# mbzuai-oryx/Video-LLaVA

Measured on NVIDIA H100. Metric: videos/sec (100-frame CLIP encode + 7B 32-tok decode), higher is better.
Workload: dtype bf16

## Files before the change

video-llava_b200/csrc/attention_tc.cu:

```cuda
#include "common.cuh"
#include "kernels.h"

#include <stdlib.h>

namespace vcl {

namespace {

constexpr int VA_WG = 2;
constexpr int VA_THREADS = VA_WG * 128;
constexpr int VA_TILE = 64 * 128;
constexpr int VA_KEY_TILES = 5;
constexpr int VA_OFF_K = 0;
constexpr int VA_OFF_VT = VA_OFF_K + VA_KEY_TILES * VA_TILE;
constexpr int VA_OFF_Q = VA_OFF_VT + VA_KEY_TILES * VA_TILE;
constexpr int VA_OFF_P = VA_OFF_Q + VA_WG * VA_TILE;
constexpr int VA_OFF_BAR = VA_OFF_P + VA_WG * VA_KEY_TILES * VA_TILE;
constexpr int VA_SMEM = VA_OFF_BAR + 64 + 1024;
static_assert(VA_SMEM <= 227 * 1024, "shared memory");

__device__ __forceinline__ uint32_t va_sw128(int row, int chunk) {
  return (uint32_t)row * 128u + (uint32_t)((chunk ^ (row & 7)) << 4);
}

__device__ __forceinline__ void named_bar_sync_wg(int id) { asm volatile("bar.sync %0, 128;" ::"r"(id) : "memory"); }

__global__ void __launch_bounds__(VA_THREADS, 1)
attn_vit_tc_kernel(const __grid_constant__ CUtensorMap tmap, const bf16* __restrict__ qkv, bf16* __restrict__ out,
                   int S, int H, int C) {
  extern __shared__ uint8_t smem_raw[];
  const uint32_t raw_addr = smem_u32(smem_raw);
  const uint32_t pad = ((raw_addr + 1023u) & ~1023u) - raw_addr;
  uint8_t* smem = smem_raw + pad;
  const uint32_t sbase = raw_addr + pad;
  const uint32_t kbar = sbase + VA_OFF_BAR;
  auto qbar = [&](int w) { return sbase + VA_OFF_BAR + 8u * (1 + w); };

  const int frame = blockIdx.x / H, h = blockIdx.x - frame * H;
  const int row0 = frame * S;
  const int wg = threadIdx.x >> 7, t = threadIdx.x & 127, lane = threadIdx.x & 31, wq = t >> 5;
  const int n_qt = (S + 63) / 64;
  const int n_kt = (S + 63) / 64;

  if (threadIdx.x == 0) {
    tma_prefetch_desc(&tmap);
    mbar_init(kbar, 1);
    for (int w = 0; w < VA_WG; ++w) mbar_init(qbar(w), 1);
    mbar_fence_init();
  }
  __syncthreads();
  if (threadIdx.x == 0) {
    mbar_arrive_expect_tx(kbar, n_kt * VA_TILE);
    for (int i = 0; i < n_kt; ++i) tma_load_2d(sbase + VA_OFF_K + i * VA_TILE, &tmap, kbar, C + h * 64, row0 + 64 * i);
    for (int w = 0; w < VA_WG && w < n_qt; ++w) {
      mbar_arrive_expect_tx(qbar(w), VA_TILE);
      tma_load_2d(sbase + VA_OFF_Q + w * VA_TILE, &tmap, qbar(w), h * 64, row0 + 64 * w);
    }
  }
  const bf16* vg = qkv + (long long)row0 * 3 * C + 2 * C + h * 64;
  for (int idx = threadIdx.x; idx < VA_KEY_TILES * 64 * 8; idx += VA_THREADS) {
    const int key = idx % (VA_KEY_TILES * 64), c = idx / (VA_KEY_TILES * 64);
    uint4 v = make_uint4(0u, 0u, 0u, 0u);
    if (key < S) v = *reinterpret_cast<const uint4*>(vg + (long long)key * 3 * C + c * 8);
    const uint32_t w4[4] = {v.x, v.y, v.z, v.w};
    uint8_t* tile = smem + VA_OFF_VT + (key >> 6) * VA_TILE;
    const int kc = (key & 63) >> 3, ke = key & 7;
#pragma unroll
    for (int e = 0; e < 8; ++e) {
      const uint16_t hv = (uint16_t)(e & 1 ? w4[e >> 1] >> 16 : w4[e >> 1] & 0xffffu);
      *reinterpret_cast<uint16_t*>(tile + va_sw128(c * 8 + e, kc) + ke * 2) = hv;
    }
  }
  asm volatile("fence.proxy.async.shared::cta;" ::: "memory");
  __syncthreads();
  mbar_wait(kbar, 0);

  const int r0 = 16 * wq + (lane >> 2), c2 = 2 * (lane & 3);
  const bool tail = S > 256;
  uint8_t* P = smem + VA_OFF_P + wg * VA_KEY_TILES * VA_TILE;
  const uint32_t p_addr = sbase + VA_OFF_P + wg * VA_KEY_TILES * VA_TILE;
  const uint32_t q_addr = sbase + VA_OFF_Q + wg * VA_TILE;
  uint32_t qphase = 0;
  float s[128], s2[16], o[32];
  for (int qt = wg; qt < n_qt; qt += VA_WG) {
    mbar_wait(qbar(wg), qphase);
    qphase ^= 1u;
#pragma unroll
    for (int i = 0; i < 128; ++i) s[i] = 0.f;
#pragma unroll
    for (int i = 0; i < 16; ++i) s2[i] = 0.f;
    wgmma_fence();
#pragma unroll
    for (int k = 0; k < 4; ++k) {
      const uint64_t ad = wgmma_desc_k_sw128(q_addr) + 2u * k;
      wgmma_bf16<256>(s, ad, wgmma_desc_k_sw128(sbase + VA_OFF_K) + 2u * k, k > 0 ? 1u : 0u);
      if (tail) wgmma_bf16<32>(s2, ad, wgmma_desc_k_sw128(sbase + VA_OFF_K + 256 * 128) + 2u * k, k > 0 ? 1u : 0u);
    }
    wgmma_commit();
    wgmma_wait<0>();
    wgmma_fence_regs(s);
    wgmma_fence_regs(s2);
    named_bar_sync_wg(1 + wg);
    if (t == 0 && qt + VA_WG < n_qt) {
      mbar_arrive_expect_tx(qbar(wg), VA_TILE);
      tma_load_2d(q_addr, &tmap, qbar(wg), h * 64, row0 + 64 * (qt + VA_WG));
    }
    auto sc = [&](float x, int key) { return key < S ? bf16r(bf16r(x) * 0.125f) : -INFINITY; };
    float m[2] = {-INFINITY, -INFINITY};
    uint32_t sp[64], sp2[8];
    auto pack_sc = [&](const float* a, int i, int key0) {
      const int hh = i & 1, col = key0 + 8 * (i >> 1) + c2;
      const float x0 = sc(a[2 * i], col), x1 = sc(a[2 * i + 1], col + 1);
      m[hh] = fmaxf(m[hh], fmaxf(x0, x1));
      return pack_bf16x2(x0, x1);
    };
    if (tail) {
#pragma unroll
      for (int i = 0; i < 8; ++i) sp2[i] = pack_sc(s2, i, 256);
    }
#pragma unroll
    for (int i = 0; i < 64; ++i) sp[i] = pack_sc(s, i, 0);
    float l[2] = {0.f, 0.f};
#pragma unroll
    for (int r = 0; r < 2; ++r) {
      m[r] = fmaxf(m[r], __shfl_xor_sync(0xffffffffu, m[r], 1));
      m[r] = fmaxf(m[r], __shfl_xor_sync(0xffffffffu, m[r], 2));
    }
    auto put_p = [&](uint32_t x2, int i, int key0) {
      const int hh = i & 1, row = r0 + 8 * hh, col = key0 + 8 * (i >> 1) + c2;
      const float p0 = exp2f((bf16lo(x2) - m[hh]) * 1.4426950408889634f);
      const float p1 = exp2f((bf16hi(x2) - m[hh]) * 1.4426950408889634f);
      l[hh] += p0 + p1;
      *reinterpret_cast<uint32_t*>(P + (col >> 6) * VA_TILE + va_sw128(row, (col & 63) >> 3) + (col & 7) * 2) =
          pack_bf16x2(p0, p1);
    };
#pragma unroll
    for (int i = 0; i < 64; ++i) put_p(sp[i], i, 0);
    if (tail) {
#pragma unroll
      for (int i = 0; i < 8; ++i) put_p(sp2[i], i, 256);
    }
    asm volatile("fence.proxy.async.shared::cta;" ::: "memory");
    named_bar_sync_wg(1 + wg);
#pragma unroll
    for (int i = 0; i < 32; ++i) o[i] = 0.f;
    wgmma_fence();
#pragma unroll
    for (int kk = 0; kk < 16; ++kk)
      wgmma_bf16<64>(o, wgmma_desc_k_sw128(p_addr + (kk >> 2) * VA_TILE) + 2u * (kk & 3),
                     wgmma_desc_k_sw128(sbase + VA_OFF_VT + (kk >> 2) * VA_TILE) + 2u * (kk & 3), kk > 0 ? 1u : 0u);
    if (tail)
      wgmma_bf16<64>(o, wgmma_desc_k_sw128(p_addr + 4 * VA_TILE), wgmma_desc_k_sw128(sbase + VA_OFF_VT + 4 * VA_TILE), 1u);
    wgmma_commit();
    wgmma_wait<0>();
    wgmma_fence_regs(o);
#pragma unroll
    for (int r = 0; r < 2; ++r) {
      l[r] += __shfl_xor_sync(0xffffffffu, l[r], 1);
      l[r] += __shfl_xor_sync(0xffffffffu, l[r], 2);
    }
#pragma unroll
    for (int hh = 0; hh < 2; ++hh) {
      const int q = qt * 64 + r0 + 8 * hh;
      if (q < S) {
        const float inv = 1.0f / l[hh];
        bf16* dst = out + (long long)(row0 + q) * C + h * 64 + c2;
#pragma unroll
        for (int j = 0; j < 8; ++j)
          *reinterpret_cast<uint32_t*>(dst + 8 * j) = pack_bf16x2(o[4 * j + 2 * hh] * inv, o[4 * j + 2 * hh + 1] * inv);
      }
    }
  }
}

}

int init_attention_tc_kernels() {
  VCL_CUDA_OK(cudaFuncSetAttribute(attn_vit_tc_kernel, cudaFuncAttributeMaxDynamicSharedMemorySize, VA_SMEM));
  return 0;
}

bool attention_vit_tc_supported(int S) {
  const bool off = getenv("VCL_VIT_ATTN_FLASH") != nullptr;
  return !off && S >= 129 && S <= 257;
}

int launch_attention_vit_tc(const bf16* qkv, bf16* out, int n_frames, int S, int H, int C, cudaStream_t stream) {
  VCL_REQUIRE(C == H * 64, "attention_vit_tc: head_dim must be 64");
  VCL_REQUIRE(S >= 129 && S <= 257, "attention_vit_tc: S=%d outside 129..257", S);
  VCL_REQUIRE(((uintptr_t)qkv % 16) == 0 && ((uintptr_t)out % 16) == 0, "attention_vit_tc: pointers must be 16-byte aligned");
  CUtensorMap tm;
  if (make_tmap_2d(&tm, qkv, (long long)n_frames * S, 3LL * C, 3LL * C, 64) != 0) return -2;
  attn_vit_tc_kernel<<<n_frames * H, VA_THREADS, VA_SMEM, stream>>>(tm, qkv, out, S, H, C);
  VCL_CUDA_OK(cudaGetLastError());
  count_launches(1);
  return 0;
}

}
```

video-llava_b200/csrc/gemm_tc.cu:

```cuda
#include "common.cuh"
#include "kernels.h"

#include <cudaTypedefs.h>

namespace vcl {

template <int BLOCK_N>
struct GemmCfg {
  static constexpr int BLOCK_M = 128;
  static constexpr int BLOCK_K = 64;
  static constexpr int A_BYTES = BLOCK_M * BLOCK_K * 2;
  static constexpr int B_BYTES = BLOCK_N * BLOCK_K * 2;
  static constexpr int STAGE_BYTES = A_BYTES + B_BYTES;
  static constexpr int OUT_PITCH = BLOCK_N * 2 + 16;
  static constexpr int OUT_BYTES = BLOCK_M * OUT_PITCH;
  static constexpr int BAR_BYTES = 256;
  static constexpr int STAGES = (BLOCK_N == 256) ? 3 : (BLOCK_N == 128 ? 5 : 8);
  static constexpr int SMEM_BYTES = STAGES * STAGE_BYTES + BAR_BYTES + OUT_BYTES + 1024;
  static_assert((2 * STAGES + 4) * 8 <= BAR_BYTES, "barrier area");
  static_assert(SMEM_BYTES <= 227 * 1024, "shared memory");
};

__device__ __forceinline__ float act_gelu_erf(float x) {
  x = bf16r(x);
  return 0.5f * x * (1.0f + erff(x * 0.70710678118654752f));
}

template <int BLOCK_N, int ACT>
__device__ __forceinline__ void gemm_epilogue_stage(const float (&acc)[BLOCK_N / 2], uint8_t* stg, int lane, int wq,
                                                    int row_base, int n_blk, const bf16* __restrict__ bias, int M,
                                                    int N, const RopeEpilogue& rp) {
  using Cfg = GemmCfg<BLOCK_N>;
  const int r0 = 16 * wq + (lane >> 2);
  const int c2 = 2 * (lane & 3);
  if constexpr (ACT == ACT_ROPE) {
    static_assert(BLOCK_N % 128 == 0, "one head (128 columns) per tile at least");
#pragma unroll
    for (int hh = 0; hh < BLOCK_N / 128; ++hh) {
      const int gh = n_blk * (BLOCK_N / 128) + hh;
      const int which = gh / rp.H;
#pragma unroll
      for (int h = 0; h < 2; ++h) {
        const int r = r0 + 8 * h;
        const int grow = row_base + r;
        int pos;
        if (rp.pack != nullptr) {
          pos = grow < M ? __ldg(pack_row(rp.pack, grow) + 1) : 0;
        } else {
          pos = rp.start_pos + (grow < M ? grow % rp.S : 0);
          if (rp.n_pad != nullptr && grow < M) pos = max(pos - __ldg(rp.n_pad + grow / rp.S), 0);
// ... 81 lines not shown
      }
    }
#pragma unroll (ACT == ACT_ROPE ? 1 : RES_INFLIGHT)
    for (int u = 0; u < RES_INFLIGHT; ++u) {
      const int r = r0 + u * RSTEP;
      if (r >= rows) break;
      const int grow = row_base + r;
      uint4 val = *reinterpret_cast<const uint4*>(stg + r * Cfg::OUT_PITCH + c * 16);
      bf16* dst = C + (long long)grow * ldc + col;
      if constexpr (ACT == ACT_ROPE) {
        const int gh = col >> 7, d = col & 127;
        const int which = gh / rp.H, head = gh - which * rp.H;
        if (which != 0) {
          int gb, col_c;
          if (rp.pack != nullptr) {
            const int2 sp = __ldg(reinterpret_cast<const int2*>(pack_row(rp.pack, grow)));
            gb = __ldg(pack_slot(rp.pack) + sp.x); col_c = sp.y;
          } else {
            gb = grow / rp.S; col_c = rp.start_pos + grow - gb * rp.S;
          }
          dst = (which == 1 ? rp.kcache : rp.vcache) + d +
                (rp.pages.table != nullptr ? kv_paged_off(rp.pages, gb, head, col_c)
                                           : (((long long)gb * rp.H + head) * rp.s_max + col_c) * 128);
        }
      } else if (RES && residual != nullptr) {
        val.x = bf16x2_add(val.x, rr[u].x); val.y = bf16x2_add(val.y, rr[u].y);
        val.z = bf16x2_add(val.z, rr[u].z); val.w = bf16x2_add(val.w, rr[u].w);
      }
      *reinterpret_cast<uint4*>(dst) = val;
    }
  }
}

template <int BLOCK_N, int ACT, int CL>
__global__ void __launch_bounds__(384, 1)
gemm_bf16_tn_kernel(const __grid_constant__ CUtensorMap tmap_a,
                    const __grid_constant__ CUtensorMap tmap_b, bf16* C, long long ldc,
                    const bf16* __restrict__ bias, const bf16* residual, long long ldr, int M,
                    int N, int K, const RopeEpilogue rope) {
  using Cfg = GemmCfg<BLOCK_N>;
  constexpr int STAGES = Cfg::STAGES;

  extern __shared__ uint8_t smem_raw[];
  const uint32_t raw_addr = smem_u32(smem_raw);
  const uint32_t pad = ((raw_addr + 1023u) & ~1023u) - raw_addr;
  uint8_t* smem = smem_raw + pad;
  const uint32_t smem_base = raw_addr + pad;

  const uint32_t bar_base = smem_base + STAGES * Cfg::STAGE_BYTES;
  auto full_bar = [&](int s) { return bar_base + 8u * s; };
  auto empty_bar = [&](int s) { return bar_base + 8u * (STAGES + s); };
  auto staged_bar = [&](int cw) { return bar_base + 8u * (2 * STAGES + cw); };
  auto drained_bar = [&](int cw) { return bar_base + 8u * (2 * STAGES + 2 + cw); };
  uint8_t* stage_out = smem + STAGES * Cfg::STAGE_BYTES + Cfg::BAR_BYTES;

  const int wg = threadIdx.x >> 7;

  if (threadIdx.x == 0) {
    tma_prefetch_desc(&tmap_a);
    tma_prefetch_desc(&tmap_b);
    for (int s = 0; s < STAGES; ++s) {
      mbar_init(full_bar(s), 1);
      mbar_init(empty_bar(s), 2 * CL);
    }
    for (int cw = 0; cw < 2; ++cw) {
      mbar_init(staged_bar(cw), 128);
      mbar_init(drained_bar(cw), STORE_THREADS);
    }
    mbar_fence_init();
  }
  __syncthreads();
  if (CL > 1) cluster_sync_all();

  const int num_m = (M + Cfg::BLOCK_M - 1) / Cfg::BLOCK_M;
  const int num_n = (N + BLOCK_N - 1) / BLOCK_N;
  const int num_k = (K + Cfg::BLOCK_K - 1) / Cfg::BLOCK_K;
  const int cta_rank = CL > 1 ? (int)cluster_ctarank() : 0;
  const int cluster_id = blockIdx.x / CL, n_clusters = gridDim.x / CL;
  const int num_tiles = ((num_m + CL - 1) / CL) * num_n;
  constexpr uint16_t MC_MASK = (uint16_t)((1u << CL) - 1u);
  constexpr int B_SLICE_ROWS = BLOCK_N / CL;

  if (wg == 0) {
    setmaxnreg_dec<56>();
    if (threadIdx.x == 0) {
      int stage = 0;
      uint32_t phase = 0;
      for (int tile = cluster_id; tile < num_tiles; tile += n_clusters) {
        const int m_blk = (tile / num_n) * CL + cta_rank, n_blk = tile % num_n;
        for (int kb = 0; kb < num_k; ++kb) {
          mbar_wait(empty_bar(stage), phase ^ 1u);
          mbar_arrive_expect_tx(full_bar(stage), Cfg::STAGE_BYTES);
          const uint32_t a_dst = smem_base + stage * Cfg::STAGE_BYTES;
          tma_load_2d(a_dst, &tmap_a, full_bar(stage), kb * Cfg::BLOCK_K, m_blk * Cfg::BLOCK_M);
          if (CL == 1) {
            tma_load_2d(a_dst + Cfg::A_BYTES, &tmap_b, full_bar(stage), kb * Cfg::BLOCK_K, n_blk * BLOCK_N);
          } else {
            tma_load_2d_mc(a_dst + Cfg::A_BYTES + cta_rank * B_SLICE_ROWS * 128, &tmap_b,
                           full_bar(stage), kb * Cfg::BLOCK_K, n_blk * BLOCK_N + cta_rank * B_SLICE_ROWS,
                           MC_MASK);
          }
          if (++stage == STAGES) { stage = 0; phase ^= 1u; }
        }
      }
    } else if (threadIdx.x >= 32) {
      const int t = threadIdx.x - 32;
      uint32_t phase = 0;
      for (int tile = cluster_id; tile < num_tiles; tile += n_clusters) {
        const int m_blk = (tile / num_n) * CL + cta_rank, n_blk = tile % num_n;
#pragma unroll 1
        for (int cw = 0; cw < 2; ++cw) {
          mbar_wait(staged_bar(cw), phase);
          gemm_epilogue_store<BLOCK_N, ACT>(stage_out + cw * 64 * Cfg::OUT_PITCH, t, m_blk * Cfg::BLOCK_M + cw * 64,
                                            n_blk, C, ldc, residual, ldr, M, N, rope);
          mbar_arrive(drained_bar(cw));
        }
        phase ^= 1u;
      }
    }
  } else {
    setmaxnreg_inc<224>();
    const int cw = wg - 1;
    const int t = threadIdx.x & 127, lane = threadIdx.x & 31, wq = t >> 5;
    uint8_t* stg = stage_out + cw * 64 * Cfg::OUT_PITCH;
    auto release = [&](int s) {
      if (t == 0) {
        if (CL == 1) {
          mbar_arrive(empty_bar(s));
        } else {
#pragma unroll
          for (int r = 0; r < CL; ++r) mbar_arrive_cluster(mapa_cluster(empty_bar(s), (uint32_t)r));
        }
      }
    };
    float acc[BLOCK_N / 2];
    int stage = 0;
    uint32_t phase = 0, out_phase = 0;
    for (int tile = cluster_id; tile < num_tiles; tile += n_clusters) {
      const int m_blk = (tile / num_n) * CL + cta_rank, n_blk = tile % num_n;
      int prev = -1;
      for (int kb = 0; kb < num_k; ++kb) {
        mbar_wait(full_bar(stage), phase);
        const uint32_t a_addr = smem_base + stage * Cfg::STAGE_BYTES;
        const uint64_t a_desc = wgmma_desc_k_sw128(a_addr + cw * 64 * 128);
        const uint64_t b_desc = wgmma_desc_k_sw128(a_addr + Cfg::A_BYTES);
        wgmma_fence();
#pragma unroll
        for (int k = 0; k < Cfg::BLOCK_K / 16; ++k) {
          wgmma_bf16<BLOCK_N>(acc, a_desc + 2u * k, b_desc + 2u * k, (kb | k) != 0 ? 1u : 0u);
        }
        wgmma_commit();
        wgmma_wait<1>();
        if (prev >= 0) release(prev);
        prev = stage;
        if (++stage == STAGES) { stage = 0; phase ^= 1u; }
      }
      wgmma_wait<0>();
      release(prev);
      wgmma_fence_regs(acc);
      if (tile != cluster_id) {
        mbar_wait(drained_bar(cw), out_phase);
        out_phase ^= 1u;
      }
      gemm_epilogue_stage<BLOCK_N, ACT>(acc, stg, lane, wq, m_blk * Cfg::BLOCK_M + cw * 64, n_blk, bias, M, N, rope);
      mbar_arrive(staged_bar(cw));
    }
  }

  __syncthreads();
  if (CL > 1) cluster_sync_all();
}

static PFN_cuTensorMapEncodeTiled_v12000 g_encode = nullptr;
static int resolve_encode() {
  if (g_encode) return 0;
  void* fn = nullptr;
  cudaDriverEntryPointQueryResult qres;
  cudaError_t e = cudaGetDriverEntryPoint("cuTensorMapEncodeTiled", &fn, cudaEnableDefault, &qres);
  if (e != cudaSuccess || fn == nullptr || qres != cudaDriverEntryPointSuccess) {
    set_last_error("cuTensorMapEncodeTiled is not available from the driver (%s)",
                   cudaGetErrorString(e));
    return -2;
  }
  g_encode = reinterpret_cast<PFN_cuTensorMapEncodeTiled_v12000>(fn);
  return 0;
}

int make_tmap_2d(CUtensorMap* out, const void* ptr, long long rows, long long cols, long long ld,
                 int box_rows) {
  if (resolve_encode() != 0) return -2;
  cuuint64_t gdim[2] = {(cuuint64_t)cols, (cuuint64_t)rows};
  cuuint64_t gstride[1] = {(cuuint64_t)ld * 2};
  cuuint32_t box[2] = {64u, (cuuint32_t)box_rows};
  cuuint32_t estr[2] = {1u, 1u};
  CUresult r = g_encode(out, CU_TENSOR_MAP_DATA_TYPE_BFLOAT16, 2, const_cast<void*>(ptr), gdim,
                        gstride, box, estr, CU_TENSOR_MAP_INTERLEAVE_NONE,
                        CU_TENSOR_MAP_SWIZZLE_128B, CU_TENSOR_MAP_L2_PROMOTION_L2_256B,
                        CU_TENSOR_MAP_FLOAT_OOB_FILL_NONE);
  if (r != CUDA_SUCCESS) {
    set_last_error("cuTensorMapEncodeTiled failed (%d) ptr=%p rows=%lld cols=%lld ld=%lld box=%d",
                   (int)r, ptr, rows, cols, ld, box_rows);
    return -2;
  }
  return 0;
}

static int g_num_sms = 0;
int device_num_sms() {
  if (g_num_sms == 0) {
    int dev = 0;
    cudaGetDevice(&dev);
    cudaDeviceGetAttribute(&g_num_sms, cudaDevAttrMultiProcessorCount, dev);
    if (g_num_sms <= 0) g_num_sms = 132;
  }
  return g_num_sms;
}

template <int BLOCK_N, int ACT, int CL>
static int launch_one(const GemmArgs& g, cudaStream_t stream) {
  using Cfg = GemmCfg<BLOCK_N>;
  auto kern = gemm_bf16_tn_kernel<BLOCK_N, ACT, CL>;
  CUtensorMap ta, tb;
  if (make_tmap_2d(&ta, g.A, g.M, g.K, g.lda, Cfg::BLOCK_M) != 0) return -2;
  if (make_tmap_2d(&tb, g.W, g.N, g.K, g.ldw, BLOCK_N / CL) != 0) return -2;
  const int num_m = (g.M + 127) / 128;
  const int num_tiles = ((num_m + CL - 1) / CL) * ((g.N + BLOCK_N - 1) / BLOCK_N);
  cudaLaunchConfig_t cfg = {};
  cfg.blockDim = dim3(384);
  cfg.dynamicSmemBytes = Cfg::SMEM_BYTES;
  cfg.stream = stream;
  cudaLaunchAttribute attr[1];
  attr[0].id = cudaLaunchAttributeClusterDimension;
  attr[0].val.clusterDim.x = CL;
  attr[0].val.clusterDim.y = 1;
  attr[0].val.clusterDim.z = 1;
  cfg.attrs = attr;
  cfg.numAttrs = CL > 1 ? 1 : 0;
  static int resident = 0;
  if (resident == 0) {
    if (CL > 1) {
      cfg.gridDim = dim3(CL);
      VCL_CUDA_OK(cudaOccupancyMaxActiveClusters(&resident, kern, &cfg));
    }
    if (resident <= 0) resident = device_num_sms() / CL;
  }
  int clusters = resident;
  if (clusters > num_tiles) clusters = num_tiles;
  if (g.max_ctas > 0 && clusters * CL > g.max_ctas) clusters = g.max_ctas / CL > 0 ? g.max_ctas / CL : 1;
  cfg.gridDim = dim3(clusters * CL);
  VCL_CUDA_OK(cudaLaunchKernelEx(&cfg, kern, ta, tb, g.C, (long long)g.ldc, g.bias, g.residual,
                                 (long long)g.ldr, g.M, g.N, g.K, g.rope));
  count_launches(1);
  return 0;
}

template <int BLOCK_N, int ACT>
static int launch_cl(const GemmArgs& g, int cl, cudaStream_t stream) {
  if (BLOCK_N >= 128) {
    if (cl == 4) return launch_one<BLOCK_N, ACT, (BLOCK_N >= 128 ? 4 : 1)>(g, stream);
    if (cl == 2) return launch_one<BLOCK_N, ACT, (BLOCK_N >= 128 ? 2 : 1)>(g, stream);
  }
  return launch_one<BLOCK_N, ACT, 1>(g, stream);
}

template <int BLOCK_N>
static int launch_act(const GemmArgs& g, int cl, cudaStream_t stream) {
  switch (g.act) {
    case ACT_NONE: return launch_cl<BLOCK_N, ACT_NONE>(g, cl, stream);
    case ACT_QGELU: return launch_cl<BLOCK_N, ACT_QGELU>(g, cl, stream);
    case ACT_GELU: return launch_cl<BLOCK_N, ACT_GELU>(g, cl, stream);
    case ACT_SWIGLU: return launch_cl<BLOCK_N, ACT_SWIGLU>(g, cl, stream);
    case ACT_ROPE:
      if constexpr (BLOCK_N >= 128) return launch_cl<BLOCK_N, ACT_ROPE>(g, cl, stream);
      break;
  }
  set_last_error("gemm: unknown activation %d", g.act);
  return -1;
}

template <int BLOCK_N, int ACT>
static int init_one() {
  VCL_CUDA_OK(cudaFuncSetAttribute(gemm_bf16_tn_kernel<BLOCK_N, ACT, 1>,
                                   cudaFuncAttributeMaxDynamicSharedMemorySize,
                                   GemmCfg<BLOCK_N>::SMEM_BYTES));
  if (BLOCK_N >= 128) {
    VCL_CUDA_OK(cudaFuncSetAttribute(gemm_bf16_tn_kernel<BLOCK_N, ACT, (BLOCK_N >= 128 ? 2 : 1)>,
                                     cudaFuncAttributeMaxDynamicSharedMemorySize,
                                     GemmCfg<BLOCK_N>::SMEM_BYTES));
    VCL_CUDA_OK(cudaFuncSetAttribute(gemm_bf16_tn_kernel<BLOCK_N, ACT, (BLOCK_N >= 128 ? 4 : 1)>,
                                     cudaFuncAttributeMaxDynamicSharedMemorySize,
                                     GemmCfg<BLOCK_N>::SMEM_BYTES));
  }
  return 0;
}
template <int BLOCK_N>
static int init_bn() {
  if (init_one<BLOCK_N, ACT_NONE>() || init_one<BLOCK_N, ACT_QGELU>() ||
      init_one<BLOCK_N, ACT_GELU>() || init_one<BLOCK_N, ACT_SWIGLU>()) return -2;
  if constexpr (BLOCK_N >= 128) {
    if (init_one<BLOCK_N, ACT_ROPE>()) return -2;
  }
  return 0;
}
int init_gemm_kernels() {
  if (resolve_encode() != 0) return -2;
  if (init_bn<256>() || init_bn<128>() || init_bn<64>() || init_bn<32>()) return -2;
  return 0;
}

int launch_gemm_bf16_tn(const GemmArgs& g, cudaStream_t stream) {
  VCL_REQUIRE(g.M > 0 && g.N > 0 && g.K > 0, "gemm: empty problem M=%d N=%d K=%d", g.M, g.N, g.K);
  VCL_REQUIRE(g.K % 64 == 0, "gemm: K=%d must be a multiple of 64", g.K);
  VCL_REQUIRE(g.N % 32 == 0, "gemm: N=%d must be a multiple of 32", g.N);
  VCL_REQUIRE(g.lda % 8 == 0 && g.ldw % 8 == 0 && g.ldc % 8 == 0, "gemm: pitches must be x8");
  VCL_REQUIRE(((uintptr_t)g.A % 16) == 0 && ((uintptr_t)g.W % 16) == 0 &&
                  ((uintptr_t)g.C % 16) == 0, "gemm: pointers must be 16-byte aligned");
  VCL_REQUIRE(g.residual == nullptr || (g.ldr % 8 == 0 && ((uintptr_t)g.residual % 16) == 0),
              "gemm: residual must be 16-byte aligned with pitch x8");
  VCL_REQUIRE(g.bias == nullptr || ((uintptr_t)g.bias % 16) == 0, "gemm: bias alignment");
  VCL_REQUIRE(!(g.act == ACT_SWIGLU && g.residual != nullptr), "gemm: swiglu takes no residual");
  if (g.act == ACT_ROPE) {
    const RopeEpilogue& r = g.rope;
    VCL_REQUIRE(r.cos_t && r.sin_t && r.kcache && r.vcache && r.S > 0 && r.H > 0, "gemm: ACT_ROPE needs the RoPE tables and the cache");
    VCL_REQUIRE(g.N == 3 * r.H * 128 && (r.pack != nullptr || g.M % r.S == 0) && r.start_pos + r.S <= r.s_max &&
                    g.bias == nullptr && g.residual == nullptr,
                "gemm: ACT_ROPE shape (N=%d, H=%d, M=%d, S=%d, start %d, cache %d)", g.N, r.H, g.M, r.S, r.start_pos, r.s_max);
    VCL_REQUIRE(((uintptr_t)r.kcache % 16) == 0 && ((uintptr_t)r.vcache % 16) == 0 && ((uintptr_t)r.cos_t % 16) == 0 &&
                    ((uintptr_t)r.sin_t % 16) == 0, "gemm: ACT_ROPE pointers must be 16-byte aligned");
  }
  int bn = g.block_n;
  int cl = g.cluster;
  if (bn == 0) {
    const int sms = device_num_sms();
    const long long mt = (g.M + 127) / 128;
    if (mt == 1) {
      bn = 256;
      while (bn > 32 && (g.N % bn != 0 || g.N / bn < sms)) bn >>= 1;
      if (g.N % bn != 0) bn = 32;
    } else if (g.N % 256 == 0 && mt * (g.N / 256) >= sms && !(g.N <= 1024 && g.K <= 1024)) {
      bn = 256;
    } else {
      bn = (g.N % 128 == 0) ? 128 : (g.N % 64 == 0) ? 64 : 32;
    }
  }
  if (cl == 0) cl = 1;
  if (cl == -2) cl = (bn == 256 || bn == 128) && g.N % bn == 0 ? 2 : 1;
  if (g.act == ACT_ROPE && g.block_n == 0 && bn < 128) bn = 128;
  VCL_REQUIRE(g.act != ACT_ROPE || bn == 128 || bn == 256, "gemm: ACT_ROPE needs 128- or 256-wide tiles (one head = 128 columns), got %d", bn);
  VCL_REQUIRE(cl == 1 || cl == 2 || cl == 4, "gemm: cluster must be 1, 2 or 4 (got %d)", cl);
  switch (bn) {
    case 256: return launch_act<256>(g, cl, stream);
    case 128: return launch_act<128>(g, cl, stream);
    case 64: return launch_act<64>(g, 1, stream);
    case 32: return launch_act<32>(g, 1, stream);
  }
  set_last_error("gemm: unsupported block_n %d", bn);
  return -1;
}

}
```

Baseline: 5.045.

## Make ViT attention persistent and warp-specialized with TMA K/V pipeline and register P

The ViT attention kernel becomes persistent, with the grid capped at the SM count. A dedicated producer warpgroup streams K, V and Q tiles through double-buffered stages and mbarriers, so loads overlap compute across (frame, head) items. V is now loaded by TMA instead of being transposed manually, and the softmax P stays in registers as the wgmma A operand instead of going through shared memory. It also adds a TAIL template, bf16x2 max/scale, and a fast ex2.approx path when the value range allows it, in exchange for more complex synchronisation and slight numeric differences.

```diff
diff --git a/video-llava_b200/csrc/attention_tc.cu b/video-llava_b200/csrc/attention_tc.cu
--- a/video-llava_b200/csrc/attention_tc.cu
+++ b/video-llava_b200/csrc/attention_tc.cu
@@ -3,157 +3,202 @@
 
 #include <stdlib.h>
 
+#include <type_traits>
+
 namespace vcl {
 
 namespace {
 
 constexpr int VA_WG = 2;
-constexpr int VA_THREADS = VA_WG * 128;
+constexpr int VA_THREADS = (VA_WG + 1) * 128;
 constexpr int VA_TILE = 64 * 128;
 constexpr int VA_KEY_TILES = 5;
-constexpr int VA_OFF_K = 0;
-constexpr int VA_OFF_VT = VA_OFF_K + VA_KEY_TILES * VA_TILE;
-constexpr int VA_OFF_Q = VA_OFF_VT + VA_KEY_TILES * VA_TILE;
-constexpr int VA_OFF_P = VA_OFF_Q + VA_WG * VA_TILE;
-constexpr int VA_OFF_BAR = VA_OFF_P + VA_WG * VA_KEY_TILES * VA_TILE;
-constexpr int VA_SMEM = VA_OFF_BAR + 64 + 1024;
+constexpr int VA_STAGES = 2;
+constexpr int VA_Q_SLOTS = 4;
+constexpr int VA_STAGE = 2 * VA_KEY_TILES * VA_TILE;
+constexpr int VA_OFF_Q = VA_STAGES * VA_STAGE;
+constexpr int VA_OFF_BAR = VA_OFF_Q + VA_Q_SLOTS * VA_TILE;
+constexpr int VA_SMEM = VA_OFF_BAR + 128 + 1024;
 static_assert(VA_SMEM <= 227 * 1024, "shared memory");
 
-__device__ __forceinline__ uint32_t va_sw128(int row, int chunk) {
-  return (uint32_t)row * 128u + (uint32_t)((chunk ^ (row & 7)) << 4);
-}
-
-__device__ __forceinline__ void named_bar_sync_wg(int id) { asm volatile("bar.sync %0, 128;" ::"r"(id) : "memory"); }
-
+__device__ __forceinline__ void wgmma_pv(float (&d)[32], uint32_t a0, uint32_t a1, uint32_t a2, uint32_t a3,
+                                         uint64_t bdesc, uint32_t accumulate) {
+  asm volatile(
+      "{\n\t.reg .pred p;\n\tsetp.ne.b32 p, %37, 0;\n\t"
+      "wgmma.mma_async.sync.aligned.m64n64k16.f32.bf16.bf16 {%0, %1, %2, %3, %4, %5, %6, %7, %8, %9, %10, %11, %12, %13, %14, %15, %16, %17, %18, %19, %20, %21, %22, %23, %24, %25, %26, %27, %28, %29, %30, %31}, {%32, %33, %34, %35}, %36, p, 1, 1, 1;\n\t}"
+      : "+f"(d[0]), "+f"(d[1]), "+f"(d[2]), "+f"(d[3]), "+f"(d[4]), "+f"(d[5]), "+f"(d[6]), "+f"(d[7]), "+f"(d[8]), "+f"(d[9]), "+f"(d[10]), "+f"(d[11]), "+f"(d[12]), "+f"(d[13]), "+f"(d[14]), "+f"(d[15]), "+f"(d[16]), "+f"(d[17]), "+f"(d[18]), "+f"(d[19]), "+f"(d[20]), "+f"(d[21]), "+f"(d[22]), "+f"(d[23]), "+f"(d[24]), "+f"(d[25]), "+f"(d[26]), "+f"(d[27]), "+f"(d[28]), "+f"(d[29]), "+f"(d[30]), "+f"(d[31])
+      : "r"(a0), "r"(a1), "r"(a2), "r"(a3), "l"(bdesc), "r"(accumulate));
+}
+
+__device__ __forceinline__ uint32_t bf16x2_max(uint32_t a, uint32_t b) {
+  __nv_bfloat162 r = __hmax2(*reinterpret_cast<__nv_bfloat162*>(&a), *reinterpret_cast<__nv_bfloat162*>(&b));
+  return *reinterpret_cast<uint32_t*>(&r);
+}
+
+__device__ __forceinline__ uint32_t bf16x2_min(uint32_t a, uint32_t b) {
+  __nv_bfloat162 r = __hmin2(*reinterpret_cast<__nv_bfloat162*>(&a), *reinterpret_cast<__nv_bfloat162*>(&b));
+  return *reinterpret_cast<uint32_t*>(&r);
+}
+__device__ __forceinline__ float ex2_approx(float x) {
+  float y;
+  asm("ex2.approx.ftz.f32 %0, %1;" : "=f"(y) : "f"(x));
+  return y;
+}
+
+template <bool TAIL>
 __global__ void __launch_bounds__(VA_THREADS, 1)
-attn_vit_tc_kernel(const __grid_constant__ CUtensorMap tmap, const bf16* __restrict__ qkv, bf16* __restrict__ out,
-                   int S, int H, int C) {
+attn_vit_tc_kernel(const __grid_constant__ CUtensorMap tmap, bf16* __restrict__ out, int S, int H, int C,
+                   int n_items) {
   extern __shared__ uint8_t smem_raw[];
   const uint32_t raw_addr = smem_u32(smem_raw);
   const uint32_t pad = ((raw_addr + 1023u) & ~1023u) - raw_addr;
-  uint8_t* smem = smem_raw + pad;
   const uint32_t sbase = raw_addr + pad;
-  const uint32_t kbar = sbase + VA_OFF_BAR;
-  auto qbar = [&](int w) { return sbase + VA_OFF_BAR + 8u * (1 + w); };
-
-  const int frame = blockIdx.x / H, h = blockIdx.x - frame * H;
-  const int row0 = frame * S;
-  const int wg = threadIdx.x >> 7, t = threadIdx.x & 127, lane = threadIdx.x & 31, wq = t >> 5;
+  auto kv_full = [&](int st) { return sbase + VA_OFF_BAR + 8u * st; };
+  auto kv_empty = [&](int st) { return sbase + VA_OFF_BAR + 8u * (VA_STAGES + st); };
+  auto q_full = [&](int sl) { return sbase + VA_OFF_BAR + 8u * (2 * VA_STAGES + sl); };
+  auto q_empty = [&](int sl) { return sbase + VA_OFF_BAR + 8u * (2 * VA_STAGES + VA_Q_SLOTS + sl); };
+
+  constexpr int n_kv = TAIL ? 5 : 4;
   const int n_qt = (S + 63) / 64;
-  const int n_kt = (S + 63) / 64;
+  const int lane = threadIdx.x & 31;
 
   if (threadIdx.x == 0) {
-    tma_prefetch_desc(&tmap);
-    mbar_init(kbar, 1);
-    for (int w = 0; w < VA_WG; ++w) mbar_init(qbar(w), 1);
+    for (int i = 0; i < VA_STAGES; ++i) {
+      mbar_init(kv_full(i), 1);
+      mbar_init(kv_empty(i), 2 * 4);
+    }
+    for (int i = 0; i < VA_Q_SLOTS; ++i) {
+      mbar_init(q_full(i), 1);
+      mbar_init(q_empty(i), 4);
+    }
     mbar_fence_init();
   }
   __syncthreads();
-  if (threadIdx.x == 0) {
-    mbar_arrive_expect_tx(kbar, n_kt * VA_TILE);
-    for (int i = 0; i < n_kt; ++i) tma_load_2d(sbase + VA_OFF_K + i * VA_TILE, &tmap, kbar, C + h * 64, row0 + 64 * i);
-    for (int w = 0; w < VA_WG && w < n_qt; ++w) {
-      mbar_arrive_expect_tx(qbar(w), VA_TILE);
-      tma_load_2d(sbase + VA_OFF_Q + w * VA_TILE, &tmap, qbar(w), h * 64, row0 + 64 * w);
-    }
+
+  if (threadIdx.x >= VA_WG * 128) {
+    setmaxnreg_dec<40>();
+    if (threadIdx.x == VA_WG * 128) {
+      const int n_mine = (n_items - (int)blockIdx.x + (int)gridDim.x - 1) / (int)gridDim.x;
+      tma_prefetch_desc(&tmap);
+      for (int j = 0, g = 0; j < n_mine; ++j) {
+        const int item = blockIdx.x + j * gridDim.x, frame = item / H, h = item - frame * H, row0 = frame * S;
+        const int st = j & 1;
+        if (j >= VA_STAGES) mbar_wait(kv_empty(st), ((j >> 1) - 1) & 1);
+        const uint32_t k_addr = sbase + st * VA_STAGE, v_addr = k_addr + VA_KEY_TILES * VA_TILE;
+        mbar_arrive_expect_tx(kv_full(st), 2 * n_kv * VA_TILE);
+        for (int i = 0; i < n_kv; ++i) {
+          tma_load_2d(k_addr + i * VA_TILE, &tmap, kv_full(st), C + h * 64, row0 + 64 * i);
+          tma_load_2d(v_addr + i * VA_TILE, &tmap, kv_full(st), 2 * C + h * 64, row0 + 64 * i);
+        }
+        for (int qt = 0; qt < n_qt; ++qt, ++g) {
+          const int sl = g & (VA_Q_SLOTS - 1);
+          if (g >= VA_Q_SLOTS) mbar_wait(q_empty(sl), ((g >> 2) - 1) & 1);
+          mbar_arrive_expect_tx(q_full(sl), VA_TILE);
+          tma_load_2d(sbase + VA_OFF_Q + sl * VA_TILE, &tmap, q_full(sl), h * 64, row0 + 64 * qt);
+        }
+      }
+    }
+    return;
   }
-  const bf16* vg = qkv + (long long)row0 * 3 * C + 2 * C + h * 64;
-  for (int idx = threadIdx.x; idx < VA_KEY_TILES * 64 * 8; idx += VA_THREADS) {
-    const int key = idx % (VA_KEY_TILES * 64), c = idx / (VA_KEY_TILES * 64);
-    uint4 v = make_uint4(0u, 0u, 0u, 0u);
-    if (key < S) v = *reinterpret_cast<const uint4*>(vg + (long long)key * 3 * C + c * 8);
-    const uint32_t w4[4] = {v.x, v.y, v.z, v.w};
-    uint8_t* tile = smem + VA_OFF_VT + (key >> 6) * VA_TILE;
-    const int kc = (key & 63) >> 3, ke = key & 7;
-#pragma unroll
-    for (int e = 0; e < 8; ++e) {
-      const uint16_t hv = (uint16_t)(e & 1 ? w4[e >> 1] >> 16 : w4[e >> 1] & 0xffffu);
-      *reinterpret_cast<uint16_t*>(tile + va_sw128(c * 8 + e, kc) + ke * 2) = hv;
-    }
-  }
-  asm volatile("fence.proxy.async.shared::cta;" ::: "memory");
-  __syncthreads();
-  mbar_wait(kbar, 0);
-
+
+  setmaxnreg_inc<232>();
+  const int n_tiles = (n_items - (int)blockIdx.x + (int)gridDim.x - 1) / (int)gridDim.x * n_qt;
+  const int wg = threadIdx.x >> 7, t = threadIdx.x & 127, wq = t >> 5;
   const int r0 = 16 * wq + (lane >> 2), c2 = 2 * (lane & 3);
-  const bool tail = S > 256;
-  uint8_t* P = smem + VA_OFF_P + wg * VA_KEY_TILES * VA_TILE;
-  const uint32_t p_addr = sbase + VA_OFF_P + wg * VA_KEY_TILES * VA_TILE;
-  const uint32_t q_addr = sbase + VA_OFF_Q + wg * VA_TILE;
-  uint32_t qphase = 0;
-  float s[128], s2[16], o[32];
-  for (int qt = wg; qt < n_qt; qt += VA_WG) {
-    mbar_wait(qbar(wg), qphase);
-    qphase ^= 1u;
-#pragma unroll
-    for (int i = 0; i < 128; ++i) s[i] = 0.f;
-#pragma unroll
-    for (int i = 0; i < 16; ++i) s2[i] = 0.f;
+  for (int g = wg; g < n_tiles; g += VA_WG) {
+    const int j = g / n_qt, qt = g - j * n_qt;
+    const int item = blockIdx.x + j * gridDim.x, frame = item / H, h = item - frame * H, row0 = frame * S;
+    const int st = j & 1, sl = g & (VA_Q_SLOTS - 1);
+    const uint32_t k_addr = sbase + st * VA_STAGE, v_addr = k_addr + VA_KEY_TILES * VA_TILE;
+    const uint32_t q_addr = sbase + VA_OFF_Q + sl * VA_TILE;
+    mbar_wait(kv_full(st), (j >> 1) & 1);
+    mbar_wait(q_full(sl), (g >> 2) & 1);
+    float s[128], s2[TAIL ? 16 : 1];
     wgmma_fence();
 #pragma unroll
     for (int k = 0; k < 4; ++k) {
       const uint64_t ad = wgmma_desc_k_sw128(q_addr) + 2u * k;
-      wgmma_bf16<256>(s, ad, wgmma_desc_k_sw128(sbase + VA_OFF_K) + 2u * k, k > 0 ? 1u : 0u);
-      if (tail) wgmma_bf16<32>(s2, ad, wgmma_desc_k_sw128(sbase + VA_OFF_K + 256 * 128) + 2u * k, k > 0 ? 1u : 0u);
+      wgmma_bf16<256>(s, ad, wgmma_desc_k_sw128(k_addr) + 2u * k, k > 0 ? 1u : 0u);
+      if constexpr (TAIL) wgmma_bf16<32>(s2, ad, wgmma_desc_k_sw128(k_addr + 256 * 128) + 2u * k, k > 0 ? 1u : 0u);
     }
     wgmma_commit();
     wgmma_wait<0>();
     wgmma_fence_regs(s);
-    wgmma_fence_regs(s2);
-    named_bar_sync_wg(1 + wg);
-    if (t == 0 && qt + VA_WG < n_qt) {
-      mbar_arrive_expect_tx(qbar(wg), VA_TILE);
-      tma_load_2d(q_addr, &tmap, qbar(wg), h * 64, row0 + 64 * (qt + VA_WG));
-    }
-    auto sc = [&](float x, int key) { return key < S ? bf16r(bf16r(x) * 0.125f) : -INFINITY; };
-    float m[2] = {-INFINITY, -INFINITY};
+    if constexpr (TAIL) wgmma_fence_regs(s2);
+    __syncwarp();
+    if (lane == 0) mbar_arrive(q_empty(sl));
+
+    constexpr int S_MIN = TAIL ? 257 : 129;
     uint32_t sp[64], sp2[8];
+    uint32_t mx[2] = {0xff80ff80u, 0xff80ff80u};
+    uint32_t mn[2] = {0x7f807f80u, 0x7f807f80u};
     auto pack_sc = [&](const float* a, int i, int key0) {
       const int hh = i & 1, col = key0 + 8 * (i >> 1) + c2;
-      const float x0 = sc(a[2 * i], col), x1 = sc(a[2 * i + 1], col + 1);
-      m[hh] = fmaxf(m[hh], fmaxf(x0, x1));
-      return pack_bf16x2(x0, x1);
+      uint32_t x2 = bf16x2_mul(pack_bf16x2(a[2 * i], a[2 * i + 1]), 0x3e003e00u);
+      mn[hh] = bf16x2_min(mn[hh], x2);
+      if (key0 + 8 * (i >> 1) + 7 >= S_MIN) {
+        if (col >= S) x2 = (x2 & 0xffff0000u) | 0xff80u;
+        if (col + 1 >= S) x2 = (x2 & 0xffffu) | 0xff800000u;
+      }
+      mx[hh] = bf16x2_max(mx[hh], x2);
+      return x2;
     };
-    if (tail) {
+    if constexpr (TAIL) {
 #pragma unroll
       for (int i = 0; i < 8; ++i) sp2[i] = pack_sc(s2, i, 256);
     }
 #pragma unroll
     for (int i = 0; i < 64; ++i) sp[i] = pack_sc(s, i, 0);
-    float l[2] = {0.f, 0.f};
+    float m[2], l[2] = {0.f, 0.f};
+    bool near = true;
 #pragma unroll
     for (int r = 0; r < 2; ++r) {
+      m[r] = fmaxf(bf16lo(mx[r]), bf16hi(mx[r]));
       m[r] = fmaxf(m[r], __shfl_xor_sync(0xffffffffu, m[r], 1));
       m[r] = fmaxf(m[r], __shfl_xor_sync(0xffffffffu, m[r], 2));
-    }
-    auto put_p = [&](uint32_t x2, int i, int key0) {
-      const int hh = i & 1, row = r0 + 8 * hh, col = key0 + 8 * (i >> 1) + c2;
-      const float p0 = exp2f((bf16lo(x2) - m[hh]) * 1.4426950408889634f);
-      const float p1 = exp2f((bf16hi(x2) - m[hh]) * 1.4426950408889634f);
+      near = near && (fminf(bf16lo(mn[r]), bf16hi(mn[r])) - m[r]) * 1.4426950408889634f >= -126.f;
+    }
+    auto p_of = [&](uint32_t x2, int i, auto bare) {
+      const int hh = i & 1;
+      const float x0 = (bf16lo(x2) - m[hh]) * 1.4426950408889634f;
+      const float x1 = (bf16hi(x2) - m[hh]) * 1.4426950408889634f;
+      const float p0 = bare ? ex2_approx(x0) : exp2f(x0), p1 = bare ? ex2_approx(x1) : exp2f(x1);
       l[hh] += p0 + p1;
-      *reinterpret_cast<uint32_t*>(P + (col >> 6) * VA_TILE + va_sw128(row, (col & 63) >> 3) + (col & 7) * 2) =
-          pack_bf16x2(p0, p1);
+      return pack_bf16x2(p0, p1);
     };
-#pragma unroll
-    for (int i = 0; i < 64; ++i) put_p(sp[i], i, 0);
-    if (tail) {
-#pragma unroll
-      for (int i = 0; i < 8; ++i) put_p(sp2[i], i, 256);
-    }
-    asm volatile("fence.proxy.async.shared::cta;" ::: "memory");
-    named_bar_sync_wg(1 + wg);
-#pragma unroll
-    for (int i = 0; i < 32; ++i) o[i] = 0.f;
+    if (qt * 64 + 16 * wq < S) {
+      if (__all_sync(0xffffffffu, near)) {
+#pragma unroll
+        for (int i = 0; i < 64; ++i) sp[i] = p_of(sp[i], i, std::true_type{});
+        if constexpr (TAIL) {
+#pragma unroll
+          for (int i = 0; i < 8; ++i) sp2[i] = p_of(sp2[i], i, std::true_type{});
+        }
+      } else {
+#pragma unroll
+        for (int i = 0; i < 64; ++i) sp[i] = p_of(sp[i], i, std::false_type{});
+        if constexpr (TAIL) {
+#pragma unroll
+          for (int i = 0; i < 8; ++i) sp2[i] = p_of(sp2[i], i, std::false_type{});
+        }
+      }
+    }
+
+    float o[32];
     wgmma_fence();
 #pragma unroll
     for (int kk = 0; kk < 16; ++kk)
-      wgmma_bf16<64>(o, wgmma_desc_k_sw128(p_addr + (kk >> 2) * VA_TILE) + 2u * (kk & 3),
-                     wgmma_desc_k_sw128(sbase + VA_OFF_VT + (kk >> 2) * VA_TILE) + 2u * (kk & 3), kk > 0 ? 1u : 0u);
-    if (tail)
-      wgmma_bf16<64>(o, wgmma_desc_k_sw128(p_addr + 4 * VA_TILE), wgmma_desc_k_sw128(sbase + VA_OFF_VT + 4 * VA_TILE), 1u);
+      wgmma_pv(o, sp[4 * kk], sp[4 * kk + 1], sp[4 * kk + 2], sp[4 * kk + 3],
+               wgmma_desc_k_sw128(v_addr + (kk >> 2) * VA_TILE + (kk & 3) * 16 * 128), kk > 0 ? 1u : 0u);
+    if constexpr (TAIL) wgmma_pv(o, sp2[0], sp2[1], sp2[2], sp2[3], wgmma_desc_k_sw128(v_addr + 4 * VA_TILE), 1u);
     wgmma_commit();
     wgmma_wait<0>();
     wgmma_fence_regs(o);
+    if (g + VA_WG >= n_tiles || (g + VA_WG) / n_qt != j) {
+      __syncwarp();
+      if (lane == 0) mbar_arrive(kv_empty(st));
+    }
+
 #pragma unroll
     for (int r = 0; r < 2; ++r) {
       l[r] += __shfl_xor_sync(0xffffffffu, l[r], 1);
@@ -166,8 +211,9 @@
         const float inv = 1.0f / l[hh];
         bf16* dst = out + (long long)(row0 + q) * C + h * 64 + c2;
 #pragma unroll
-        for (int j = 0; j < 8; ++j)
-          *reinterpret_cast<uint32_t*>(dst + 8 * j) = pack_bf16x2(o[4 * j + 2 * hh] * inv, o[4 * j + 2 * hh + 1] * inv);
+        for (int j8 = 0; j8 < 8; ++j8)
+          *reinterpret_cast<uint32_t*>(dst + 8 * j8) =
+              pack_bf16x2(o[4 * j8 + 2 * hh] * inv, o[4 * j8 + 2 * hh + 1] * inv);
       }
     }
   }
@@ -176,7 +222,8 @@
 }
 
 int init_attention_tc_kernels() {
-  VCL_CUDA_OK(cudaFuncSetAttribute(attn_vit_tc_kernel, cudaFuncAttributeMaxDynamicSharedMemorySize, VA_SMEM));
+  VCL_CUDA_OK(cudaFuncSetAttribute(attn_vit_tc_kernel<false>, cudaFuncAttributeMaxDynamicSharedMemorySize, VA_SMEM));
+  VCL_CUDA_OK(cudaFuncSetAttribute(attn_vit_tc_kernel<true>, cudaFuncAttributeMaxDynamicSharedMemorySize, VA_SMEM));
   return 0;
 }
 
@@ -191,7 +238,15 @@
   VCL_REQUIRE(((uintptr_t)qkv % 16) == 0 && ((uintptr_t)out % 16) == 0, "attention_vit_tc: pointers must be 16-byte aligned");
   CUtensorMap tm;
   if (make_tmap_2d(&tm, qkv, (long long)n_frames * S, 3LL * C, 3LL * C, 64) != 0) return -2;
-  attn_vit_tc_kernel<<<n_frames * H, VA_THREADS, VA_SMEM, stream>>>(tm, qkv, out, S, H, C);
+  int dev = 0, sms = 0;
+  VCL_CUDA_OK(cudaGetDevice(&dev));
+  VCL_CUDA_OK(cudaDeviceGetAttribute(&sms, cudaDevAttrMultiProcessorCount, dev));
+  const int items = n_frames * H;
+  const int grid = items < sms ? items : sms;
+  if (S > 256)
+    attn_vit_tc_kernel<true><<<grid, VA_THREADS, VA_SMEM, stream>>>(tm, out, S, H, C, items);
+  else
+    attn_vit_tc_kernel<false><<<grid, VA_THREADS, VA_SMEM, stream>>>(tm, out, S, H, C, items);
   VCL_CUDA_OK(cudaGetLastError());
   count_launches(1);
   return 0;
```

New measurement: 5.142 (median of 6 runs). 1.9% higher.

## Add 64-row unit schedule for GEMM and M-fast tile order for small M

Applied to the files above, without the earlier changes.

Adds an opt-in GEMM schedule (cluster=-1) that splits work into 64-row by BLOCK_N units, divides them evenly across CTAs and pairs consecutive units per pass, loading a second B strip when the pair crosses strips. For small M (num_m<=4) the default path now walks tiles M-fastest so that CTAs sharing a weight strip run together, and the 256-wide tile choice drops its K condition. An environment override for tile and cluster is also added. The unit path is meant to reduce wave-quantization tail imbalance, at the cost of more complex barrier bookkeeping and extra B traffic.

```diff
diff --git a/video-llava_b200/csrc/gemm_tc.cu b/video-llava_b200/csrc/gemm_tc.cu
--- a/video-llava_b200/csrc/gemm_tc.cu
+++ b/video-llava_b200/csrc/gemm_tc.cu
@@ -2,20 +2,23 @@
 #include "kernels.h"
 
 #include <cudaTypedefs.h>
+#include <cstdio>
+#include <cstdlib>
 
 namespace vcl {
 
-template <int BLOCK_N>
+template <int BLOCK_N, bool UNITS = false>
 struct GemmCfg {
   static constexpr int BLOCK_M = 128;
   static constexpr int BLOCK_K = 64;
   static constexpr int A_BYTES = BLOCK_M * BLOCK_K * 2;
   static constexpr int B_BYTES = BLOCK_N * BLOCK_K * 2;
-  static constexpr int STAGE_BYTES = A_BYTES + B_BYTES;
+  static constexpr int STAGE_BYTES = A_BYTES + (UNITS ? 2 : 1) * B_BYTES;
   static constexpr int OUT_PITCH = BLOCK_N * 2 + 16;
   static constexpr int OUT_BYTES = BLOCK_M * OUT_PITCH;
   static constexpr int BAR_BYTES = 256;
-  static constexpr int STAGES = (BLOCK_N == 256) ? 3 : (BLOCK_N == 128 ? 5 : 8);
+  static constexpr int STAGES = UNITS ? (227 * 1024 - BAR_BYTES - OUT_BYTES - 1024) / STAGE_BYTES
+                                      : (BLOCK_N == 256) ? 3 : (BLOCK_N == 128 ? 5 : 8);
   static constexpr int SMEM_BYTES = STAGES * STAGE_BYTES + BAR_BYTES + OUT_BYTES + 1024;
   static_assert((2 * STAGES + 4) * 8 <= BAR_BYTES, "barrier area");
   static_assert(SMEM_BYTES <= 227 * 1024, "shared memory");
@@ -163,13 +166,14 @@
   }
 }
 
-template <int BLOCK_N, int ACT, int CL>
+template <int BLOCK_N, int ACT, int CL, bool UNITS = false>
 __global__ void __launch_bounds__(384, 1)
 gemm_bf16_tn_kernel(const __grid_constant__ CUtensorMap tmap_a,
                     const __grid_constant__ CUtensorMap tmap_b, bf16* C, long long ldc,
                     const bf16* __restrict__ bias, const bf16* residual, long long ldr, int M,
                     int N, int K, const RopeEpilogue rope) {
-  using Cfg = GemmCfg<BLOCK_N>;
+  static_assert(!UNITS || CL == 1, "the unit schedule runs without a cluster");
+  using Cfg = GemmCfg<BLOCK_N, UNITS>;
   constexpr int STAGES = Cfg::STAGES;
 
   extern __shared__ uint8_t smem_raw[];
@@ -211,21 +215,62 @@
   const int num_tiles = ((num_m + CL - 1) / CL) * num_n;
   constexpr uint16_t MC_MASK = (uint16_t)((1u << CL) - 1u);
   constexpr int B_SLICE_ROWS = BLOCK_N / CL;
+  const int num_rb = (M + 63) / 64;
+  const long long num_units = (long long)num_rb * num_n;
+  const int it_begin = UNITS ? (int)(blockIdx.x * num_units / gridDim.x) : cluster_id;
+  const int it_end = UNITS ? (int)((blockIdx.x + 1) * num_units / gridDim.x) : num_tiles;
+  const int it_step = UNITS ? 2 : n_clusters;
+  const bool m_fast = CL == 1 && num_m <= 4;
+  struct Pass {
+    int row0, row1, strip0, strip1;
+    bool has1, two_b;
+    __device__ int row(int cw) const { return cw ? row1 : row0; }
+    __device__ int strip(int cw) const { return cw ? strip1 : strip0; }
+  };
+  auto pass_of = [&](int it) {
+    Pass p;
+    if constexpr (UNITS) {
+      p.has1 = it + 1 < it_end;
+      p.strip0 = it / num_rb;
+      p.row0 = (it - p.strip0 * num_rb) * 64;
+      p.strip1 = (it + 1) / num_rb;
+      p.row1 = (it + 1 - p.strip1 * num_rb) * 64;
+      p.two_b = p.has1 && p.strip1 != p.strip0;
+    } else if (m_fast) {
+      p.row0 = (it % num_m) * Cfg::BLOCK_M; p.row1 = p.row0 + 64;
+      p.strip0 = p.strip1 = it / num_m;
+      p.has1 = true; p.two_b = false;
+    } else {
+      const int m_blk = (it / num_n) * CL + cta_rank;
+      p.row0 = m_blk * Cfg::BLOCK_M; p.row1 = p.row0 + 64;
+      p.strip0 = p.strip1 = it % num_n;
+      p.has1 = true; p.two_b = false;
+    }
+    return p;
+  };
 
   if (wg == 0) {
     setmaxnreg_dec<56>();
     if (threadIdx.x == 0) {
       int stage = 0;
       uint32_t phase = 0;
-      for (int tile = cluster_id; tile < num_tiles; tile += n_clusters) {
-        const int m_blk = (tile / num_n) * CL + cta_rank, n_blk = tile % num_n;
+      for (int it = it_begin; it < it_end; it += it_step) {
+        const Pass p = pass_of(it);
+        const int n_blk = p.strip0;
+        const uint32_t bytes = UNITS ? (p.has1 ? 2 : 1) * (Cfg::A_BYTES / 2) + (p.two_b ? 2 : 1) * Cfg::B_BYTES
+                                     : Cfg::STAGE_BYTES;
         for (int kb = 0; kb < num_k; ++kb) {
           mbar_wait(empty_bar(stage), phase ^ 1u);
-          mbar_arrive_expect_tx(full_bar(stage), Cfg::STAGE_BYTES);
+          mbar_arrive_expect_tx(full_bar(stage), bytes);
           const uint32_t a_dst = smem_base + stage * Cfg::STAGE_BYTES;
-          tma_load_2d(a_dst, &tmap_a, full_bar(stage), kb * Cfg::BLOCK_K, m_blk * Cfg::BLOCK_M);
+          tma_load_2d(a_dst, &tmap_a, full_bar(stage), kb * Cfg::BLOCK_K, p.row0);
+          if (UNITS && p.has1)
+            tma_load_2d(a_dst + Cfg::A_BYTES / 2, &tmap_a, full_bar(stage), kb * Cfg::BLOCK_K, p.row1);
           if (CL == 1) {
             tma_load_2d(a_dst + Cfg::A_BYTES, &tmap_b, full_bar(stage), kb * Cfg::BLOCK_K, n_blk * BLOCK_N);
+            if (p.two_b)
+              tma_load_2d(a_dst + Cfg::A_BYTES + Cfg::B_BYTES, &tmap_b, full_bar(stage), kb * Cfg::BLOCK_K,
+                          p.strip1 * BLOCK_N);
           } else {
             tma_load_2d_mc(a_dst + Cfg::A_BYTES + cta_rank * B_SLICE_ROWS * 128, &tmap_b,
                            full_bar(stage), kb * Cfg::BLOCK_K, n_blk * BLOCK_N + cta_rank * B_SLICE_ROWS,
@@ -237,13 +282,13 @@
     } else if (threadIdx.x >= 32) {
       const int t = threadIdx.x - 32;
       uint32_t phase = 0;
-      for (int tile = cluster_id; tile < num_tiles; tile += n_clusters) {
-        const int m_blk = (tile / num_n) * CL + cta_rank, n_blk = tile % num_n;
+      for (int it = it_begin; it < it_end; it += it_step) {
+        const Pass p = pass_of(it);
 #pragma unroll 1
-        for (int cw = 0; cw < 2; ++cw) {
+        for (int cw = 0; cw < (p.has1 ? 2 : 1); ++cw) {
           mbar_wait(staged_bar(cw), phase);
-          gemm_epilogue_store<BLOCK_N, ACT>(stage_out + cw * 64 * Cfg::OUT_PITCH, t, m_blk * Cfg::BLOCK_M + cw * 64,
-                                            n_blk, C, ldc, residual, ldr, M, N, rope);
+          gemm_epilogue_store<BLOCK_N, ACT>(stage_out + cw * 64 * Cfg::OUT_PITCH, t, p.row(cw), p.strip(cw), C, ldc,
+                                            residual, ldr, M, N, rope);
           mbar_arrive(drained_bar(cw));
         }
         phase ^= 1u;
@@ -267,14 +312,23 @@
     float acc[BLOCK_N / 2];
     int stage = 0;
     uint32_t phase = 0, out_phase = 0;
-    for (int tile = cluster_id; tile < num_tiles; tile += n_clusters) {
-      const int m_blk = (tile / num_n) * CL + cta_rank, n_blk = tile % num_n;
+    for (int it = it_begin; it < it_end; it += it_step) {
+      const Pass p = pass_of(it);
+      if (cw == 1 && !p.has1) {
+        for (int kb = 0; kb < num_k; ++kb) {
+          mbar_wait(full_bar(stage), phase);
+          release(stage);
+          if (++stage == STAGES) { stage = 0; phase ^= 1u; }
+        }
+        continue;
+      }
+      const uint32_t b_off = Cfg::A_BYTES + (p.two_b && cw == 1 ? Cfg::B_BYTES : 0);
       int prev = -1;
       for (int kb = 0; kb < num_k; ++kb) {
         mbar_wait(full_bar(stage), phase);
         const uint32_t a_addr = smem_base + stage * Cfg::STAGE_BYTES;
         const uint64_t a_desc = wgmma_desc_k_sw128(a_addr + cw * 64 * 128);
-        const uint64_t b_desc = wgmma_desc_k_sw128(a_addr + Cfg::A_BYTES);
+        const uint64_t b_desc = wgmma_desc_k_sw128(a_addr + b_off);
         wgmma_fence();
 #pragma unroll
         for (int k = 0; k < Cfg::BLOCK_K / 16; ++k) {
@@ -289,11 +343,11 @@
       wgmma_wait<0>();
       release(prev);
       wgmma_fence_regs(acc);
-      if (tile != cluster_id) {
+      if (it != it_begin) {
         mbar_wait(drained_bar(cw), out_phase);
         out_phase ^= 1u;
       }
-      gemm_epilogue_stage<BLOCK_N, ACT>(acc, stg, lane, wq, m_blk * Cfg::BLOCK_M + cw * 64, n_blk, bias, M, N, rope);
+      gemm_epilogue_stage<BLOCK_N, ACT>(acc, stg, lane, wq, p.row(cw), p.strip(cw), bias, M, N, rope);
       mbar_arrive(staged_bar(cw));
     }
   }
@@ -347,15 +401,16 @@
   return g_num_sms;
 }
 
-template <int BLOCK_N, int ACT, int CL>
+template <int BLOCK_N, int ACT, int CL, bool UNITS = false>
 static int launch_one(const GemmArgs& g, cudaStream_t stream) {
-  using Cfg = GemmCfg<BLOCK_N>;
-  auto kern = gemm_bf16_tn_kernel<BLOCK_N, ACT, CL>;
+  using Cfg = GemmCfg<BLOCK_N, UNITS>;
+  auto kern = gemm_bf16_tn_kernel<BLOCK_N, ACT, CL, UNITS>;
   CUtensorMap ta, tb;
-  if (make_tmap_2d(&ta, g.A, g.M, g.K, g.lda, Cfg::BLOCK_M) != 0) return -2;
+  if (make_tmap_2d(&ta, g.A, g.M, g.K, g.lda, UNITS ? 64 : Cfg::BLOCK_M) != 0) return -2;
   if (make_tmap_2d(&tb, g.W, g.N, g.K, g.ldw, BLOCK_N / CL) != 0) return -2;
   const int num_m = (g.M + 127) / 128;
-  const int num_tiles = ((num_m + CL - 1) / CL) * ((g.N + BLOCK_N - 1) / BLOCK_N);
+  const int num_n = (g.N + BLOCK_N - 1) / BLOCK_N;
+  const int num_tiles = UNITS ? (int)(((long long)(g.M + 63) / 64 * num_n + 1) / 2) : ((num_m + CL - 1) / CL) * num_n;
   cudaLaunchConfig_t cfg = {};
   cfg.blockDim = dim3(384);
   cfg.dynamicSmemBytes = Cfg::SMEM_BYTES;
@@ -387,6 +442,9 @@
 
 template <int BLOCK_N, int ACT>
 static int launch_cl(const GemmArgs& g, int cl, cudaStream_t stream) {
+  if constexpr (BLOCK_N == 128 || BLOCK_N == 64) {
+    if (cl == -1) return launch_one<BLOCK_N, ACT, 1, true>(g, stream);
+  }
   if (BLOCK_N >= 128) {
     if (cl == 4) return launch_one<BLOCK_N, ACT, (BLOCK_N >= 128 ? 4 : 1)>(g, stream);
     if (cl == 2) return launch_one<BLOCK_N, ACT, (BLOCK_N >= 128 ? 2 : 1)>(g, stream);
@@ -414,6 +472,11 @@
   VCL_CUDA_OK(cudaFuncSetAttribute(gemm_bf16_tn_kernel<BLOCK_N, ACT, 1>,
                                    cudaFuncAttributeMaxDynamicSharedMemorySize,
                                    GemmCfg<BLOCK_N>::SMEM_BYTES));
+  if constexpr (BLOCK_N == 128 || BLOCK_N == 64) {
+    VCL_CUDA_OK(cudaFuncSetAttribute(gemm_bf16_tn_kernel<BLOCK_N, ACT, 1, true>,
+                                     cudaFuncAttributeMaxDynamicSharedMemorySize,
+                                     GemmCfg<BLOCK_N, true>::SMEM_BYTES));
+  }
   if (BLOCK_N >= 128) {
     VCL_CUDA_OK(cudaFuncSetAttribute(gemm_bf16_tn_kernel<BLOCK_N, ACT, (BLOCK_N >= 128 ? 2 : 1)>,
                                      cudaFuncAttributeMaxDynamicSharedMemorySize,
@@ -461,6 +524,12 @@
   }
   int bn = g.block_n;
   int cl = g.cluster;
+  static const int2 tile_env = [] {
+    int2 t = make_int2(0, 0);
+    if (const char* e = getenv("VCL_GEMM_TILE")) sscanf(e, "%d,%d", &t.x, &t.y);
+    return t;
+  }();
+  if (bn == 0 && cl == 0 && tile_env.x != 0) { bn = tile_env.x; cl = tile_env.y; }
   if (bn == 0) {
     const int sms = device_num_sms();
     const long long mt = (g.M + 127) / 128;
@@ -468,21 +537,23 @@
       bn = 256;
       while (bn > 32 && (g.N % bn != 0 || g.N / bn < sms)) bn >>= 1;
       if (g.N % bn != 0) bn = 32;
-    } else if (g.N % 256 == 0 && mt * (g.N / 256) >= sms && !(g.N <= 1024 && g.K <= 1024)) {
+    } else if (g.N % 256 == 0 && mt * (g.N / 256) >= sms && g.N > 1024) {
       bn = 256;
     } else {
       bn = (g.N % 128 == 0) ? 128 : (g.N % 64 == 0) ? 64 : 32;
     }
   }
   if (cl == 0) cl = 1;
+  if (cl == -1 && bn == 0) bn = g.N % 128 == 0 ? 128 : 64;
+  VCL_REQUIRE(cl != -1 || bn == 128 || bn == 64, "gemm: the 64-row unit schedule takes 128- or 64-wide strips, got %d", bn);
   if (cl == -2) cl = (bn == 256 || bn == 128) && g.N % bn == 0 ? 2 : 1;
   if (g.act == ACT_ROPE && g.block_n == 0 && bn < 128) bn = 128;
   VCL_REQUIRE(g.act != ACT_ROPE || bn == 128 || bn == 256, "gemm: ACT_ROPE needs 128- or 256-wide tiles (one head = 128 columns), got %d", bn);
-  VCL_REQUIRE(cl == 1 || cl == 2 || cl == 4, "gemm: cluster must be 1, 2 or 4 (got %d)", cl);
+  VCL_REQUIRE(cl == 1 || cl == 2 || cl == 4 || cl == -1, "gemm: cluster must be 1, 2, 4 or -1 (got %d)", cl);
   switch (bn) {
     case 256: return launch_act<256>(g, cl, stream);
     case 128: return launch_act<128>(g, cl, stream);
-    case 64: return launch_act<64>(g, 1, stream);
+    case 64: return launch_act<64>(g, cl == -1 ? -1 : 1, stream);
     case 32: return launch_act<32>(g, 1, stream);
   }
   set_last_error("gemm: unsupported block_n %d", bn);
```

Result: faster. 5.047 before, 5.162 after, median of 6 (+2.3%).
